# Eurus-Holmes/VAG-NMT

Measured on AMD Instinct MI355X. Metric: training sentence-pairs/sec (Multi30K en->de, B=64), higher is better.
Workload: dtype f32; 1 GPU; configs[1]: multimodal en->de train step, B=64/GPU, Ts=Tt=40, E=256, H=512, S=512, I=2048, Vs=8507, V=9391, dropout 0.3/0.5/0.5, tied emb, teacher_force_ratio=1; global_batch=64, parallelism=dp1, hip_graph=True

## Files before the change

vag-nmt_amd/csrc/api.hip:

```cpp
#include "../../include/vag_nmt.h"
#include "api_shared.h"
#include <cstring>

static thread_local VagCallCtx g_base_ctx;
static thread_local VagCallCtx* g_active_ctx = nullptr;
VagCallCtx& vag_ctx() { return g_active_ctx ? *g_active_ctx : g_base_ctx; }
VagCallScope::VagCallScope(VagCallCtx& c) : ctx(c), prev(g_active_ctx) { g_active_ctx = &c; }
VagCallScope::~VagCallScope() {
    (void)vag_loss_defer_flush();
    if (ctx.leaf_on) vag_leaf_drop();
    g_active_ctx = prev;
}

VagOptions& vag_opt() {
    static VagOptions o;
    return o;
}

int vag_version(void) { return 330; }

int vag_set_option(const char* name, int64_t value) {
    VAG_CHECK_ARG(name != nullptr);
    VagOptions& o = vag_opt();
    const struct { const char* n; int* p; } ints[] = {
// ... 545 lines not shown
    return vag_surface_expand_launch(rows, R, L, off, chars, V, out, C, lens, S_(stream));
}
int vag_chrf_supported(int64_t Nh, int64_t Ch, int64_t Nr, int64_t Cr) { return vag_chrf_supported_host(Nh, Ch, Nr, Cr); }
int vag_chrf_max_chars(void) { return vag_chrf_max_chars_host(); }
int vag_chrf_select(const int32_t* hchars, const int32_t* hlens, const int32_t* rchars, const int32_t* rlens, const float* weights,
                    int64_t B, int64_t Nh, int64_t Ch, int64_t Nr, int64_t Cr, int32_t* matches, float* util, float* expected,
                    int64_t* best, vag_stream_t stream) {
    return vag_chrf_select_launch(hchars, hlens, rchars, rlens, weights, B, Nh, Ch, Nr, Cr, matches, util, expected, best, S_(stream));
}

int vag_mrt_weights(const float* nll, const float* cost, const float* valid, int64_t B, int64_t Tt, int64_t N, float alpha, float scale,
                    float* inv_cnt, float* q, float* risk, vag_stream_t stream) {
    VAG_CHECK_ARG(risk != nullptr);
    return vag_mrt_weights_launch(nll, cost, valid, B, Tt, N, alpha, scale, inv_cnt, q, risk, nullptr, 0.f, 0, S_(stream));
}
int vag_mrt_pack(const int64_t* cand, int64_t G, int64_t Nc, int64_t L, const int64_t* gold, int64_t Tg, int include_gold, int64_t* tgt,
                 int64_t Tt, float* valid, vag_stream_t stream) {
    return vag_mrt_pack_launch(cand, G, Nc, L, gold, Tg, include_gold, tgt, Tt, valid, S_(stream));
}

int vag_clip_adam_flat(float* p, float* g, float* m, float* v, int64_t n, int nseg, const int64_t* seg_off,
                       const float* seg_lr, const float* seg_wd, float clip, float grad_scale, float beta1, float beta2,
                       float eps, int zero_grad, int32_t* step, float* norm_out, void* scratch, const float* lr_dev,
                       vag_stream_t stream) {
    return vag_clip_adam_launch(p, g, m, v, n, nseg, seg_off, seg_lr, seg_wd, clip, grad_scale, beta1, beta2, eps, zero_grad,
                                step, norm_out, scratch, lr_dev, S_(stream));
}

int vag_clip_adam_flat_ema(float* p, float* g, float* m, float* v, int64_t n, int nseg, const int64_t* seg_off,
                           const float* seg_lr, const float* seg_wd, float clip, float grad_scale, float beta1, float beta2,
                           float eps, int zero_grad, int32_t* step, float* norm_out, void* scratch, const float* lr_dev,
                           float* ema, float ema_decay, int ema_warmup, vag_stream_t stream) {
    return vag_clip_adam_ema_launch(p, g, m, v, n, nseg, seg_off, seg_lr, seg_wd, clip, grad_scale, beta1, beta2, eps, zero_grad,
                                    step, norm_out, scratch, lr_dev, ema, ema_decay, ema_warmup, S_(stream));
}

int vag_swap_flat(float* a, float* b, int64_t n, vag_stream_t stream) { return vag_swap_flat_launch(a, b, n, S_(stream)); }

int vag_clip_adam_shard(float* p, float* g, float* m, float* v, int64_t n, int nseg, const int64_t* seg_off, const float* seg_lr,
                        const float* seg_wd, float clip, float grad_scale, float beta1, float beta2, float eps, int zero_grad,
                        int32_t* step, float* norm_out, void* scratch, const float* lr_dev, int64_t lo, int64_t hi, int phase,
                        double* sumsq, vag_stream_t stream) {
    return vag_clip_adam_shard_launch(p, g, m, v, n, nseg, seg_off, seg_lr, seg_wd, clip, grad_scale, beta1, beta2, eps, zero_grad,
                                      step, norm_out, scratch, lr_dev, lo, hi, phase, sumsq, S_(stream));
}

int vag_copy4(const void* const* src, void* const* dst, const int64_t* bytes, int n, vag_stream_t stream) {
    return vag_copy4_launch(src, dst, bytes, n, S_(stream));
}

int vag_recurrence_supported(int kind, int64_t B, int64_t Ts, int64_t Tt, int64_t H) {
    if (kind == 0) return vag_enc_persistent_ok(B, Ts, H) ? 1 : 0;
    if (kind == 1) return vag_dec_persistent_ok(B, Ts, Tt, H) ? 1 : 0;
    return 0;
}
int vag_persistent_timeouts(void) { return vag_persistent_timeouts_read(); }
int vag_attn_energy_probe(const float* a, const float* b, int64_t n, float* out, vag_stream_t stream) {
    return vag_attn_energy_probe_launch(a, b, n, out, S_(stream));
}
int64_t vag_handoff_planes_floats(int64_t B, int64_t Ts, int64_t Tt, int64_t H) {
    const int64_t e = vag_enc_bwd_planes_floats(B, Ts, H), d = vag_dec_bwd_planes_floats(B, Tt, H);
    const int64_t f = vag_enc_fwd_planes_floats(B, Ts, H) + vag_dec_fwd_planes_floats(B, Tt, H);
    return std::max(std::max(e, d), f);
}
int vag_set_handoff_planes(float* buf, int64_t floats) {
    VAG_CHECK_ARG((buf == nullptr || (floats > 0 && aligned16(buf))));
    g_base_ctx.handoff_planes = buf;
    g_base_ctx.handoff_floats = buf ? floats : 0;
    return VAG_OK;
}
int vag_set_operator_guard(void* guard) {
    VAG_CHECK_ARG((reinterpret_cast<uintptr_t>(guard) & 3) == 0);
    g_base_ctx.guard = reinterpret_cast<unsigned*>(guard);
    return VAG_OK;
}
int vag_gemm_group_plan(int n, const int64_t* M, const int64_t* N, const int64_t* K, const int* accumulate, int* split,
                        int* order) {
    return vag_gemm_group_plan_host(n, M, N, K, accumulate, split, order);
}
int vag_gemm_plan(int64_t M, int64_t N, int64_t K, int a_kc, int b_kc, int vec, float beta, int act, int c_half, int a_bf16,
                  int rowsum, int planes, int* plan) {
    return vag_gemm_plan_host(M, N, K, a_kc, b_kc, vec, beta, act, c_half, a_bf16, rowsum, planes, plan);
}
int vag_recurrence_time(int kind, double* ms_total, int* launches) { return vag_persistent_time_read(kind, ms_total, launches); }
int64_t vag_recurrence_sync_words(int kind, int64_t B, int64_t T) {
    return kind == 0 ? vag_enc_persistent_sync_words(B, T) : vag_dec_persistent_sync_words(B, T);
}
int vag_dropout_mask(const uint64_t* rng, int which, int64_t n, float p, float* out, vag_stream_t stream) {
    VAG_CHECK_ARG(which >= 1 && which <= 3);
    return vag_dropout_mask_launch(rng, which, n, p, out, S_(stream));
}
int vag_rng_advance(uint64_t* rng, vag_stream_t stream) { return vag_rng_advance_launch(rng, S_(stream)); }
```

vag-nmt_amd/csrc/persist.hip:

```cpp
#include "kernels.h"
#include "gemm_shared.h"
#include <algorithm>
#include <atomic>
#include <mutex>

namespace {

typedef unsigned __attribute__((address_space(1))) gu32;
#define RLX_AGENT __ATOMIC_RELAXED, __HIP_MEMORY_SCOPE_AGENT

constexpr unsigned SPIN_LIMIT = 1u << 19;
__device__ unsigned g_persist_timeouts;
__device__ unsigned g_persist_guard[2];
__device__ __forceinline__ void note_timeout(unsigned* err, unsigned* guard) {
    __hip_atomic_store((gu32*)err, 1u, RLX_AGENT);
    __hip_atomic_store((gu32*)guard, 1u, RLX_AGENT);
    atomicAdd(guard + 1, 1u);
    atomicAdd(&g_persist_timeouts, 1u);
}

struct EncPArgs {
    const float* xp;
    const float* W[2];
    const float* bias[2];
    const int* lengths;
    float* hst;
    float* gates;
    float* enc;
    unsigned* cnt;
    unsigned* err;
    unsigned* guard;
    unsigned spin;
    const uint64_t* rng;
    float p_ctx;
    int B, Ts, H, RT, CS;
    int rt0, RTP;
    char* pl;
};

template <int N> __device__ __forceinline__ void ld_rows_sc1(const float* p, float4 (&a)[N], float4 (&b)[N]);
template <> __device__ __forceinline__ void ld_rows_sc1<1>(const float* p, float4 (&a)[1], float4 (&b)[1]) {
    asm volatile("global_load_dwordx4 %0, %2, off sc1\n\tglobal_load_dwordx4 %1, %2, off offset:16 sc1\n\ts_waitcnt vmcnt(0)"
                 : "=&v"(a[0]), "=&v"(b[0]) : "v"(p) : "memory");
}
template <> __device__ __forceinline__ void ld_rows_sc1<2>(const float* p, float4 (&a)[2], float4 (&b)[2]) {
    asm volatile("global_load_dwordx4 %0, %4, off sc1\n\tglobal_load_dwordx4 %1, %4, off offset:16 sc1\n\t"
                 "global_load_dwordx4 %2, %4, off offset:128 sc1\n\tglobal_load_dwordx4 %3, %4, off offset:144 sc1\n\t"
                 "s_waitcnt vmcnt(0)"
                 : "=&v"(a[0]), "=&v"(b[0]), "=&v"(a[1]), "=&v"(b[1]) : "v"(p) : "memory");
}
template <> __device__ __forceinline__ void ld_rows_sc1<3>(const float* p, float4 (&a)[3], float4 (&b)[3]) {
    asm volatile("global_load_dwordx4 %0, %6, off sc1\n\tglobal_load_dwordx4 %1, %6, off offset:16 sc1\n\t"
                 "global_load_dwordx4 %2, %6, off offset:128 sc1\n\tglobal_load_dwordx4 %3, %6, off offset:144 sc1\n\t"
                 "global_load_dwordx4 %4, %6, off offset:256 sc1\n\tglobal_load_dwordx4 %5, %6, off offset:272 sc1\n\t"
                 "s_waitcnt vmcnt(0)"
                 : "=&v"(a[0]), "=&v"(b[0]), "=&v"(a[1]), "=&v"(b[1]), "=&v"(a[2]), "=&v"(b[2]) : "v"(p) : "memory");
}
template <> __device__ __forceinline__ void ld_rows_sc1<4>(const float* p, float4 (&a)[4], float4 (&b)[4]) {
    asm volatile("global_load_dwordx4 %0, %8, off sc1\n\tglobal_load_dwordx4 %1, %8, off offset:16 sc1\n\t"
                 "global_load_dwordx4 %2, %8, off offset:128 sc1\n\tglobal_load_dwordx4 %3, %8, off offset:144 sc1\n\t"
                 "global_load_dwordx4 %4, %8, off offset:256 sc1\n\tglobal_load_dwordx4 %5, %8, off offset:272 sc1\n\t"
                 "global_load_dwordx4 %6, %8, off offset:384 sc1\n\tglobal_load_dwordx4 %7, %8, off offset:400 sc1\n\t"
// ... 517 lines not shown
    unsigned* err;
    unsigned* guard;
    unsigned spin;
    int B, Ts, H, RT, CS;
    int rt0, RTP;
    char* pl;
};
template <int KS, bool PL>
__global__ __launch_bounds__(512, 1) void enc_bwd_persistent_kernel(EncBArgs a) {
    __shared__ __attribute__((aligned(16))) float lds[21504];
    const int wg = blockIdx.x;
    const int cs = wg % a.CS, rt = a.rt0 + (wg / a.CS) % a.RTP, d = wg / (a.CS * a.RTP);
    const int lane = threadIdx.x & 63, wave = threadIdx.x >> 6;
    const int H = a.H, B = a.B, Ts = a.Ts, K = 3 * H;
    const int m0 = rt * 16, u0 = cs * 16;
    const int fr = lane & 15, fg = lane >> 4;
    const int kbase = wave * (K >> 3);
    const int64_t BH = (int64_t)B * H;
    bf16x8 wf[KS][3];
    {
        const float* WT = a.WT[d] + (int64_t)(u0 + fr) * K + kbase + 8 * fg;
#pragma unroll
        for (int s = 0; s < KS; ++s) split8(*reinterpret_cast<const float4*>(WT + 32 * s), *reinterpret_cast<const float4*>(WT + 32 * s + 4), wf[s]);
    }
    const int erow = lane >> 2, equad = lane & 3, eslot = erow + 16 * equad;
    const int em = m0 + erow, eu = u0 + 4 * equad;
    const bool eok = wave == 0 && em < B;
    const int len = eok ? a.lengths[em] : 0;
    float4 carry = make_float4(0.f, 0.f, 0.f, 0.f);
    float* dghd = a.dgh + (int64_t)d * Ts * B * K;
    const char* pld = PL ? a.pl + ((int64_t)d * Ts * a.RT + rt) * pl_block_bytes(K) : nullptr;
    const int64_t pl_step = (int64_t)a.RT * pl_block_bytes(K);
    const int pl_ld = __builtin_amdgcn_readfirstlane(wave) * KS * PL_KSTEP_BYTES;
    const int pl_st = (u0 >> 5) * PL_KSTEP_BYTES, pl_gate = (H >> 5) * PL_KSTEP_BYTES;
    const unsigned pl_so = pl_slot_off(lane >> 2, u0 + 4 * (lane & 3));
    gu32* cnt = (gu32*)(a.cnt + ((int64_t)d * a.RT + rt) * Ts);
    const int lrow = min(m0 + ld_row(lane), B - 1);
    const int src4 = ld_src4(lane);
    float4* red = reinterpret_cast<float4*>(lds);
    bool dead = false;
    const int64_t ld_add = (int64_t)Ts * 2 * H;

    for (int k = Ts - 1; k >= 0; --k) {
        const int t = d == 0 ? k : Ts - 1 - k;
        float4 sv[4], hp, e4;
        if (eok) {
            const int64_t o = (int64_t)em * H + eu;
            const float* g = a.gates + ((int64_t)(d * Ts + k) * 4) * BH + o;
#pragma unroll
            for (int q = 0; q < 4; ++q) sv[q] = *reinterpret_cast<const float4*>(g + q * BH);
            hp = *reinterpret_cast<const float4*>(a.hst + ((int64_t)d * (Ts + 1) + k) * BH + o);
            e4 = *reinterpret_cast<const float4*>(a.d_enc + (int64_t)em * ld_add + (int64_t)t * 2 * H + d * H + eu);
        }
        float4 dh = carry;
        if (k < Ts - 1) {
            if (threadIdx.x == 0 && !dead) {
                unsigned spins = 0;
                while (__hip_atomic_load(cnt + (k + 1), RLX_AGENT) < (unsigned)a.CS) {
                    if (++spins > a.spin) { note_timeout(a.err, a.guard); dead = true; break; }
                }
            }
            __syncthreads();
            f32x4 acc = {0.f, 0.f, 0.f, 0.f};
            if (PL) {
                u32x4 gf[3 * KS];
                ld_planes_sc1<KS>(pld + (k + 1) * pl_step + pl_ld, 16u * lane, gf);
                acc = mma6_planes<KS>(wf, gf, acc);
            } else {
                float4 ga[KS], gb[KS];
                ld_rows_sc1<KS>(dghd + ((int64_t)(k + 1) * B + lrow) * K + kbase + 8 * (lane & 3), ga, gb);
#pragma unroll
                for (int s = 0; s < KS; ++s) {
                    bf16x8 hf[3];
                    split8(perm4(ga[s], src4), perm4(gb[s], src4), hf);
                    acc = mma6(wf[s], hf, acc);
                }
            }
            red[wave * 64 + lane] = make_float4(acc[0], acc[1], acc[2], acc[3]);
            __syncthreads();
            if (wave == 0) {
#pragma unroll
                for (int w = 0; w < 8; ++w) {
                    const float4 o = red[w * 64 + eslot];
                    dh.x += o.x; dh.y += o.y; dh.z += o.z; dh.w += o.w;
                }
            }
        }
        if (PL && wave == 0 && !eok) {
#pragma unroll
            for (int g = 0; g < 3; ++g) st_planes4(pld + k * pl_step + pl_st + g * pl_gate, pl_so, make_float4(0.f, 0.f, 0.f, 0.f));
        }
        if (eok) {
            const bool active = t < len;
            float dhv[4] = {dh.x, dh.y, dh.z, dh.w};
            float gi[3][4], gh[3][4], cy[4];
            if (!active) {
#pragma unroll
                for (int q = 0; q < 4; ++q) { gi[0][q] = gi[1][q] = gi[2][q] = gh[0][q] = gh[1][q] = gh[2][q] = 0.f; cy[q] = dhv[q]; }
            } else {
                const float ev[4] = {e4.x, e4.y, e4.z, e4.w};
                const float r_[4] = {sv[0].x, sv[0].y, sv[0].z, sv[0].w}, z_[4] = {sv[1].x, sv[1].y, sv[1].z, sv[1].w};
                const float n_[4] = {sv[2].x, sv[2].y, sv[2].z, sv[2].w}, hn[4] = {sv[3].x, sv[3].y, sv[3].z, sv[3].w};
                const float hpv[4] = {hp.x, hp.y, hp.z, hp.w};
#pragma unroll
                for (int q = 0; q < 4; ++q) {
                    float e = ev[q];
                    if (a.rng && a.p_ctx > 0.f)
                        e *= vag_drop_mul(a.rng, VAG_DROP_ENC_CTX, (uint64_t)em * ld_add + (uint64_t)t * 2 * H + d * H + eu + q, a.p_ctx);
                    const float x = dhv[q] + e;
                    const float dn_pre = x * (1.f - z_[q]) * (1.f - n_[q] * n_[q]);
                    const float dz_pre = x * (hpv[q] - n_[q]) * z_[q] * (1.f - z_[q]);
                    const float dr_pre = dn_pre * hn[q] * r_[q] * (1.f - r_[q]);
                    gi[0][q] = dr_pre; gi[1][q] = dz_pre; gi[2][q] = dn_pre;
                    gh[0][q] = dr_pre; gh[1][q] = dz_pre; gh[2][q] = dn_pre * r_[q];
                    cy[q] = x * z_[q];
                }
            }
            carry = make_float4(cy[0], cy[1], cy[2], cy[3]);
            float* gho = dghd + ((int64_t)k * B + em) * K + eu;
#pragma unroll
            for (int g = 0; g < 3; ++g) {
                const float4 x = make_float4(gh[g][0], gh[g][1], gh[g][2], gh[g][3]);
                if (PL) st_planes4(pld + k * pl_step + pl_st + g * pl_gate, pl_so, x);
                else st_sc1_f4(gho + g * H, x);
            }
            asm volatile("s_waitcnt vmcnt(0)" ::: "memory");
            if (lane == 0) __hip_atomic_fetch_add(cnt + k, 1u, RLX_AGENT);
            if (PL) {
#pragma unroll
                for (int g = 0; g < 3; ++g) *reinterpret_cast<float4*>(gho + g * H) = make_float4(gh[g][0], gh[g][1], gh[g][2], gh[g][3]);
            }
            float* gio = a.d_xp + ((int64_t)t * B + em) * 6 * H + d * 3 * H + eu;
#pragma unroll
            for (int g = 0; g < 3; ++g) *reinterpret_cast<float4*>(gio + g * H) = make_float4(gi[g][0], gi[g][1], gi[g][2], gi[g][3]);
        }
    }
}

struct EncWBArgs {
    const vag_half* WT16[2];
    const float* d_enc;
    const float* gates;
    const float* hst;
    const int* lengths;
    const uint64_t* rng; float p_ctx;
    float* d_xp;
    float* dgh;
    vag_half* gx;
    unsigned* cnt;
    unsigned* err;
    unsigned* guard;
    unsigned spin;
    int B, Ts, H, RG, CS;
};
template <> __device__ __forceinline__ void ld16_sc1<6>(const vag_half* p, u32x4 (&v)[6]) {
    asm volatile("global_load_dwordx4 %0, %6, off sc1\n\tglobal_load_dwordx4 %1, %6, off offset:64 sc1\n\t"
                 "global_load_dwordx4 %2, %6, off offset:128 sc1\n\tglobal_load_dwordx4 %3, %6, off offset:192 sc1\n\t"
                 "global_load_dwordx4 %4, %6, off offset:256 sc1\n\tglobal_load_dwordx4 %5, %6, off offset:320 sc1\n\t"
                 "s_waitcnt vmcnt(0)"
                 : "=&v"(v[0]), "=&v"(v[1]), "=&v"(v[2]), "=&v"(v[3]), "=&v"(v[4]), "=&v"(v[5]) : "v"(p) : "memory");
}
// ... 208 lines not shown
                 "global_load_dwordx4 %10, %28, off offset:128 sc1\n\tglobal_load_dwordx4 %11, %28, off offset:144 sc1\n\t"
                 "global_load_dwordx4 %12, %28, off offset:256 sc1\n\tglobal_load_dwordx4 %13, %28, off offset:272 sc1\n\t"
                 "global_load_dwordx4 %14, %28, off offset:384 sc1\n\tglobal_load_dwordx4 %15, %28, off offset:400 sc1\n\t"
                 "global_load_dwordx4 %16, %28, off offset:512 sc1\n\tglobal_load_dwordx4 %17, %28, off offset:528 sc1\n\t"
                 "global_load_dwordx4 %18, %28, off offset:640 sc1\n\tglobal_load_dwordx4 %19, %28, off offset:656 sc1\n\t"
                 "s_waitcnt vmcnt(0)"
                 : "=&v"(a0), "=&v"(a1), "=&v"(a2), "=&v"(a3), "=&v"(b0), "=&v"(b1), "=&v"(b2), "=&v"(b3),
                   "=&v"(a[0]), "=&v"(b[0]), "=&v"(a[1]), "=&v"(b[1]), "=&v"(a[2]), "=&v"(b[2]), "=&v"(a[3]), "=&v"(b[3]),
                   "=&v"(a[4]), "=&v"(b[4]), "=&v"(a[5]), "=&v"(b[5])
                 : "v"(p0), "v"(p01), "v"(p02), "v"(p03), "v"(p1), "v"(p11), "v"(p12), "v"(p13), "v"(rows) : "memory");
    v0 = (a0 + a1) + (a2 + a3);
    v1 = (b0 + b1) + (b2 + b3);
}

__device__ __forceinline__ void ld_acc_shards_and_rows3(const float* p0, const float* p1, int64_t stride, float& v0, float& v1,
                                                        const float* rows, float4 (&a)[3], float4 (&b)[3]) {
    float a0, a1, a2, a3, b0, b1, b2, b3;
    const float *p02 = p0 + 2 * stride, *p12 = p1 + 2 * stride;
    const float *p01 = p0 + stride, *p03 = p02 + stride, *p11 = p1 + stride, *p13 = p12 + stride;
    asm volatile("global_load_dword %0, %14, off sc1\n\tglobal_load_dword %1, %15, off sc1\n\t"
                 "global_load_dword %2, %16, off sc1\n\tglobal_load_dword %3, %17, off sc1\n\t"
                 "global_load_dword %4, %18, off sc1\n\tglobal_load_dword %5, %19, off sc1\n\t"
                 "global_load_dword %6, %20, off sc1\n\tglobal_load_dword %7, %21, off sc1\n\t"
                 "global_load_dwordx4 %8, %22, off sc1\n\tglobal_load_dwordx4 %9, %22, off offset:16 sc1\n\t"
                 "global_load_dwordx4 %10, %22, off offset:128 sc1\n\tglobal_load_dwordx4 %11, %22, off offset:144 sc1\n\t"
                 "global_load_dwordx4 %12, %22, off offset:256 sc1\n\tglobal_load_dwordx4 %13, %22, off offset:272 sc1\n\t"
                 "s_waitcnt vmcnt(0)"
                 : "=&v"(a0), "=&v"(a1), "=&v"(a2), "=&v"(a3), "=&v"(b0), "=&v"(b1), "=&v"(b2), "=&v"(b3),
                   "=&v"(a[0]), "=&v"(b[0]), "=&v"(a[1]), "=&v"(b[1]), "=&v"(a[2]), "=&v"(b[2])
                 : "v"(p0), "v"(p01), "v"(p02), "v"(p03), "v"(p1), "v"(p11), "v"(p12), "v"(p13), "v"(rows) : "memory");
    v0 = (a0 + a1) + (a2 + a3);
    v1 = (b0 + b1) + (b2 + b3);
}
__device__ __forceinline__ void ld_acc_shards_and_rows(const float* p0, const float* p1, int64_t stride, float& v0, float& v1,
                                                       const float* rows, float4 (&a)[6], float4 (&b)[6]) {
    ld_acc_shards_and_rows6(p0, p1, stride, v0, v1, rows, a, b);
}
__device__ __forceinline__ void ld_acc_shards_and_rows(const float* p0, const float* p1, int64_t stride, float& v0, float& v1,
                                                       const float* rows, float4 (&a)[3], float4 (&b)[3]) {
    ld_acc_shards_and_rows3(p0, p1, stride, v0, v1, rows, a, b);
}

constexpr int DEC_WGS = 64;
template <int WGS>
__device__ __forceinline__ void dec_slice_map(int mode, int rt0, int& i, int& rt) {
    const int bx = blockIdx.x % WGS;
    rt = rt0 + blockIdx.x / WGS;
    int g = mode == 1 ? 8 : (mode == 2 ? 2 : (mode == 3 ? 4 : 1));
    if (g > WGS / 8) g = WGS / 8;
    i = (bx & 7) * g + ((bx >> 3) % g) + 8 * g * (bx / (8 * g));
}
constexpr int ACC_SHARDS = 4;
constexpr int DEC_U = 8;

constexpr int DEC_E = 4 * DEC_WGS;
__device__ __forceinline__ unsigned long long cand_key(float v, int idx) {
    const unsigned u = __builtin_bit_cast(unsigned, v);
    return ((unsigned long long)(u ^ ((u >> 31) ? 0xffffffffu : 0x80000000u)) << 32) | (unsigned long long)(0xffffffffu - (unsigned)idx);
}

template <bool FREE, int WGS = DEC_WGS, bool PL = false>
__global__ __launch_bounds__(512, 1) void dec_fwd_persistent_kernel(DecPArgs a) {
    extern __shared__ __attribute__((aligned(16))) float dlds[];
    static_assert(WGS == 64 || (WGS == 32 && !FREE), "H = 512 (both forms) or H = 256 (teacher-forced form)");
    static_assert(!(PL && FREE), "the free-running form keeps the fp32 hand-off");
    constexpr int H = WGS * DEC_U, C = 2 * H, Q = C + 3 * H, KS = H / 256;
    constexpr int E = DEC_E;
    int i, rt;
    dec_slice_map<WGS>(a.xcd_map, a.rt0, i, rt);
    const int lane = threadIdx.x & 63, wave = threadIdx.x >> 6;
    const int B = a.B, Ts = a.Ts, Tt = a.Tt;
    const int m0 = rt * 16, u0 = i * DEC_U;
    const int fr = lane & 15, fg = lane >> 4;
    const int kbase = wave * (H >> 3);
    const int64_t BH = (int64_t)B * H;
    float4* red = reinterpret_cast<float4*>(dlds);
    float* pe_s = dlds + 6144;
    float* ew_s = pe_s + 16 * Ts * 16;
    float* sc_s = ew_s + 16 * Ts * 24;
    float* gi_s = sc_s + 16 * Ts;
    float* hp_s = gi_s + 16 * 24;
    float* bs_s = hp_s + 16 * 24;
    float* hs_s = bs_s + 80;
    float* v_s = hs_s + 256;
    float* mk_s = v_s + C;
    float* q_s = mk_s + 16 * Ts;
    float* cw_s = q_s + 256;
    float* hb_s = cw_s + 64;
    int* tok_s = reinterpret_cast<int*>(hb_s + 16);
    float* ew2_s = reinterpret_cast<float*>(tok_s + 16);
    unsigned long long* cb_s = reinterpret_cast<unsigned long long*>(q_s);
    bf16x8* tm_s = reinterpret_cast<bf16x8*>(red);

#ifdef VAG_LAB
#define VAG_PSTAMP(k) do { if (!FREE && a.dbg && blockIdx.x == 0 && threadIdx.x == 0) a.dbg[Tt * 8 + (k)] = __builtin_amdgcn_s_memrealtime(); } while (0)
#else
#define VAG_PSTAMP(k) do { } while (0)
#endif
    VAG_PSTAMP(0);
#ifdef VAG_LAB
    if (!FREE && a.dbg && threadIdx.x == 0 && rt < 8) {
        if (i == 0) a.dbg[(Tt + 1) * 8 + rt] = __builtin_amdgcn_s_memrealtime();
        if (i == WGS - 1) a.dbg[(Tt + 3) * 8 + rt] = __builtin_amdgcn_s_memrealtime();
    }
#endif
    bf16x8 w1[KS][2][3], w2[KS][3][3];
// ... 373 lines not shown
                    ho[q] = (1.f - zz[q]) * nn[q] + zz[q] * hpv[q];
                }
                const float4 h1v = tag4(make_float4(ho[0], ho[1], ho[2], ho[3]));
                *reinterpret_cast<float4*>(hs_s + fr * 8 + 4 * hq) = h1v;
                const int64_t o = (int64_t)em * H + eu;
                st_sc1_f4(a.h1 + (int64_t)t * BH + o, h1v);
                if (!VAG_TAGGED) asm volatile("s_waitcnt vmcnt(0)" ::: "memory");
                if (VAG_TAGGED && tx == 0) arrive(c2 + t * CNT_WORDS, i);
                float* sv = a.g1 + (int64_t)t * 4 * BH + o;
                *reinterpret_cast<float4*>(sv) = make_float4(rr[0], rr[1], rr[2], rr[3]);
                *reinterpret_cast<float4*>(sv + BH) = make_float4(zz[0], zz[1], zz[2], zz[3]);
                *reinterpret_cast<float4*>(sv + 2 * BH) = make_float4(nn[0], nn[1], nn[2], nn[3]);
                *reinterpret_cast<float4*>(sv + 3 * BH) = make_float4(gh[0], gh[1], gh[2], gh[3]);
            }
            if (tx == 0 && (!VAG_TAGGED || !eok)) arrive(c2 + t * CNT_WORDS, i);
        }
        VAG_STAMP(2);
        wait_count(c2 + t * CNT_WORDS, PER_SHARD, a.err, a.guard, a.spin, dead);
        VAG_STAMP(3);
        bf16x8 hf2[KS][3];
        if constexpr (PL) {
            u32x4 gf[3 * KS];
            ld_planes_marked<KS>(plb + t * pl_step + pl_ld, 16u * lane, gf, a.spin, dead, a.err, a.guard);
#pragma unroll
            for (int s = 0; s < 3 * KS; ++s) hf2[s / 3][s % 3] = __builtin_bit_cast(bf16x8, gf[s]);
        } else {
            ld_rows_tagged<KS>(a.h1 + ((int64_t)t * B + lrow) * H + kbase + 8 * (lane & 3), ha, hb, a.spin, dead, a.err, a.guard);
#pragma unroll
            for (int s = 0; s < KS; ++s) { ha[s] = perm4(ha[s], src4); hb[s] = perm4(hb[s], src4); }
        }
        {
            f32x4 acc = {0.f, 0.f, 0.f, 0.f};
#pragma unroll
            for (int s = 0; s < KS; ++s) {
                if constexpr (!PL) split8(ha[s], hb[s], hf2[s]);
                acc = mma6(w2[s][0], hf2[s], acc);
            }
            red[(wave * 3 + 0) * 64 + lane] = make_float4(acc[0], acc[1], acc[2], acc[3]);
        }
        __syncthreads();
        if (wave == 0) {
            float4 qv = make_float4(0, 0, 0, 0);
#pragma unroll
            for (int w = 0; w < 8; ++w) {
                const float4 x0 = red[(w * 3 + 0) * 64 + lane];
                qv.x += x0.x; qv.y += x0.y; qv.z += x0.z; qv.w += x0.w;
            }
            if (m0 + fr < B) *reinterpret_cast<float4*>(a.qhp + ((int64_t)t * B + m0 + fr) * Q + 16 * i + 4 * fg) = qv;
            *reinterpret_cast<float4*>(q_s + fr * 16 + 4 * fg) =
                make_float4(vag_energy_exp(qv.x), vag_energy_exp(qv.y), vag_energy_exp(qv.z), vag_energy_exp(qv.w));
        }
        __syncthreads();
        {
            const int cq = tx & 3;
            const float4 vq = *reinterpret_cast<const float4*>(v_s + 16 * i + 4 * cq);
            for (int P = tx >> 2; P < 16 * Ts; P += 128) {
                const int r = P / Ts;
                const float4 pv = reinterpret_cast<const float4*>(pe_s)[P * 4 + cq];
                const float4 qq = *reinterpret_cast<const float4*>(q_s + r * 16 + 4 * cq);
                float acc = vq.x * vag_energy_tanh(pv.x, qq.x) + vq.y * vag_energy_tanh(pv.y, qq.y) + vq.z * vag_energy_tanh(pv.z, qq.z) +
                            vq.w * vag_energy_tanh(pv.w, qq.w);
                acc = quad_sum(acc);
                if (cq == 0 && m0 + r < B)
                    atomicAdd(a.psc + (((int64_t)t * ACC_SHARDS + (i & (ACC_SHARDS - 1))) * B + m0 + r) * Ts + (P - r * Ts), acc);
            }
        }
        {
            f32x4 acc[2] = {{0.f, 0.f, 0.f, 0.f}, {0.f, 0.f, 0.f, 0.f}};
#pragma unroll
            for (int s = 0; s < KS; ++s) {
                acc[0] = mma6(w2[s][1], hf2[s], acc[0]);
                acc[1] = mma6(w2[s][2], hf2[s], acc[1]);
            }
            red[(wave * 3 + 1) * 64 + lane] = make_float4(acc[0][0], acc[0][1], acc[0][2], acc[0][3]);
            red[(wave * 3 + 2) * 64 + lane] = make_float4(acc[1][0], acc[1][1], acc[1][2], acc[1][3]);
        }
        VAG_STAMP(4);
        asm volatile("s_waitcnt vmcnt(0)" ::: "memory");
        __syncthreads();
        if (tx == 0) arrive(c4 + t * CNT_WORDS, i);
        VAG_STAMP(5);
        if (ep) {
            float4 hp2[3] = {make_float4(0, 0, 0, 0), make_float4(0, 0, 0, 0), make_float4(0, 0, 0, 0)};
#pragma unroll
            for (int w = 0; w < 8; ++w) {
                const float4 x0 = red[(w * 3 + 1) * 64 + hq * 16 + fr], x1 = red[(w * 3 + 1) * 64 + (2 + hq) * 16 + fr];
                const float4 x2 = red[(w * 3 + 2) * 64 + hq * 16 + fr];
                hp2[0].x += x0.x; hp2[0].y += x0.y; hp2[0].z += x0.z; hp2[0].w += x0.w;
                hp2[1].x += x1.x; hp2[1].y += x1.y; hp2[1].z += x1.z; hp2[1].w += x1.w;
                hp2[2].x += x2.x; hp2[2].y += x2.y; hp2[2].z += x2.z; hp2[2].w += x2.w;
            }
#pragma unroll
            for (int g = 0; g < 3; ++g) {
                const float4 bb = *reinterpret_cast<const float4*>(bs_s + 24 + g * 8 + 4 * hq);
                hp2[g].x += bb.x; hp2[g].y += bb.y; hp2[g].z += bb.z; hp2[g].w += bb.w;
                *reinterpret_cast<float4*>(hp_s + fr * 24 + g * 8 + 4 * hq) = hp2[g];
                if (eok) *reinterpret_cast<float4*>(a.qhp + ((int64_t)t * B + em) * Q + C + g * H + eu) = hp2[g];
            }
        }
        VAG_STAMP(6);
        wait_count(c4 + t * CNT_WORDS, PER_SHARD, a.err, a.guard, a.spin, dead);
        VAG_STAMP(7);
        for (int x0 = tx; x0 < 16 * Ts; x0 += 1024) {
            const int x1 = x0 + 512;
            const int r0 = x0 / Ts, r1 = min(x1, 16 * Ts - 1) / Ts;
            const float* p0 = a.psc + ((int64_t)t * ACC_SHARDS * B + min(m0 + r0, B - 1)) * Ts + (x0 - r0 * Ts);
            const float* p1 = a.psc + ((int64_t)t * ACC_SHARDS * B + min(m0 + r1, B - 1)) * Ts + (min(x1, 16 * Ts - 1) - r1 * Ts);
            float v0, v1;
            ld_acc_shards(p0, p1, (int64_t)B * Ts, v0, v1);
            sc_s[x0] = mk_s[x0] == 0.f ? -INFINITY : v0;
            if (x1 < 16 * Ts) sc_s[x1] = mk_s[x1] == 0.f ? -INFINITY : v1;
        }
        __syncthreads();
        for (int r = wave; r < 16; r += 8) {
            float mx = -INFINITY;
            for (int sp = lane; sp < Ts; sp += 64) mx = fmaxf(mx, sc_s[r * Ts + sp]);
            mx = wave_max(mx);
            float sum = 0.f;
            for (int sp = lane; sp < Ts; sp += 64) sum += __expf(sc_s[r * Ts + sp] - mx);
            sum = wave_sum(sum);
            const float inv = 1.f / sum;
            for (int sp = lane; sp < Ts; sp += 64) {
                const float al = __expf(sc_s[r * Ts + sp] - mx) * inv;
                sc_s[r * Ts + sp] = al;
                if (((r * Ts + sp) & (WGS - 1)) == i && m0 + r < B) a.alpha[((int64_t)t * B + m0 + r) * Ts + sp] = al;
            }
        }
        __syncthreads();
        if (tx < 16 * 24) {
            const int r = tx / 24, col = tx - r * 24;
            const float* al = sc_s + r * Ts;
            const float* ew = ew_s + (int64_t)r * Ts * 24 + col;
            float s0 = 0.f, s1 = 0.f;
            int sp = 0;
            for (; sp + 1 < Ts; sp += 2) { s0 += al[sp] * ew[sp * 24]; s1 += al[sp + 1] * ew[(sp + 1) * 24]; }
            if (sp < Ts) s0 += al[sp] * ew[sp * 24];
            gi_s[tx] = s0 + s1;
        } else if (FREE && tx < 16 * 24 + 64) {
            const int x = tx - 16 * 24, r = x >> 2, col = x & 3;
            const float* al = sc_s + r * Ts;
            const float* ew = ew2_s + (int64_t)r * Ts * 4 + col;
            float s0 = 0.f, s1 = 0.f;
            int sp = 0;
            for (; sp + 1 < Ts; sp += 2) { s0 += al[sp] * ew[sp * 4]; s1 += al[sp + 1] * ew[(sp + 1) * 4]; }
            if (sp < Ts) s0 += al[sp] * ew[sp * 4];
            cw_s[x] = s0 + s1;
        }
        __syncthreads();
        if constexpr (PL) {
            if (ep2 && !eok2) st_planes2_marked(plb + (Tt + t) * pl_step + pl_st, pl_so + 4 * eh, 0.f, 0.f);
            if (eok2) {
                const int e8 = 4 * hq + 2 * eh;
                float gi[3][2], bi[3][2], hh[3][2];
#pragma unroll
                for (int g = 0; g < 3; ++g) {
                    const float2 x = *reinterpret_cast<const float2*>(gi_s + fr * 24 + g * 8 + e8);
                    const float2 y = *reinterpret_cast<const float2*>(bs_s + 48 + g * 8 + e8);
                    const float2 z = *reinterpret_cast<const float2*>(hp_s + fr * 24 + g * 8 + e8);
                    gi[g][0] = x.x; gi[g][1] = x.y;
                    bi[g][0] = y.x; bi[g][1] = y.y;
                    hh[g][0] = z.x; hh[g][1] = z.y;
                }
                const float2 h1v = *reinterpret_cast<const float2*>(hs_s + fr * 8 + e8);
                const float h1a[2] = {h1v.x, h1v.y};
                float rr[2], zz[2], nn[2], ho[2];
#pragma unroll
                for (int q = 0; q < 2; ++q) {
                    rr[q] = vag_sigmoid(gi[0][q] + bi[0][q] + hh[0][q]);
                    zz[q] = vag_sigmoid(gi[1][q] + bi[1][q] + hh[1][q]);
                    nn[q] = vag_tanh(gi[2][q] + bi[2][q] + rr[q] * hh[2][q]);
                    ho[q] = (1.f - zz[q]) * nn[q] + zz[q] * h1a[q];
                }
                const float2 h2v = make_float2(tag1(ho[0]), tag1(ho[1]));
                *reinterpret_cast<float2*>(hs_s + 128 + fr * 8 + e8) = h2v;
                st_planes2_marked(plb + (Tt + t) * pl_step + pl_st, pl_so + 4 * eh, h2v.x, h2v.y);
                if (tx == 0) arrive(c1 + t * CNT_WORDS, i);
                const int64_t o = (int64_t)em * H + eu2;
                *reinterpret_cast<float2*>(a.h2_all + (int64_t)t * BH + o) = h2v;
                float* sv = a.g2 + (int64_t)t * 4 * BH + o;
                *reinterpret_cast<float2*>(sv) = make_float2(rr[0], rr[1]);
                *reinterpret_cast<float2*>(sv + BH) = make_float2(zz[0], zz[1]);
                *reinterpret_cast<float2*>(sv + 2 * BH) = make_float2(nn[0], nn[1]);
                *reinterpret_cast<float2*>(sv + 3 * BH) = make_float2(hh[2][0], hh[2][1]);
            }
            if (tx == 0 && !eok2) arrive(c1 + t * CNT_WORDS, i);
        }
        if (!PL && eok) {
            float gi[3][4];
#pragma unroll
            for (int g = 0; g < 3; ++g) {
                const float4 x = *reinterpret_cast<const float4*>(gi_s + fr * 24 + g * 8 + 4 * hq);
                gi[g][0] = x.x; gi[g][1] = x.y; gi[g][2] = x.z; gi[g][3] = x.w;
            }
            float bi[3][4], hh[3][4];
#pragma unroll
            for (int g = 0; g < 3; ++g) {
                const float4 x = *reinterpret_cast<const float4*>(bs_s + 48 + g * 8 + 4 * hq);
                const float4 y = *reinterpret_cast<const float4*>(hp_s + fr * 24 + g * 8 + 4 * hq);
                bi[g][0] = x.x; bi[g][1] = x.y; bi[g][2] = x.z; bi[g][3] = x.w;
// ... 180 lines not shown
    auto red4 = [&](float (&x)[4]) {
        float4 sum = red[hq * 16 + fr];
#pragma unroll
        for (int w = 1; w < 8; ++w) {
            const float4 o = red[w * 64 + hq * 16 + fr];
            sum.x += o.x; sum.y += o.y; sum.z += o.z; sum.w += o.w;
        }
        x[0] = sum.x; x[1] = sum.y; x[2] = sum.z; x[3] = sum.w;
    };
    auto hid_load = [&](int t, int c, bf16x8 (&wf)[3][3], u32x4 (&gf)[9]) {
        unsigned w2o = pl_w2_off;
        asm volatile("" : "+v"(w2o));
        const char* pw = pl_w2 + w2o;
#pragma unroll
        for (int s = 0; s < 3; ++s)
#pragma unroll
            for (int p = 0; p < 3; ++p)
                wf[s][p] = *reinterpret_cast<const bf16x8*>(pw + (3 * c + s) * PL_W2_KSTEP_BYTES + p * PL_W2_PLANE_BYTES);
        ld_planes_sc1<3>(pl_g2 + t * pl_g1_step + KC * pl_wave + c * (3 * PL_KSTEP_BYTES), 16u * lane, gf);
    };

    VAG_BPSTAMP(1);
    if (ep) {
        if (eok) {
            const float4 d = *reinterpret_cast<const float4*>(a.d_h2_all + (int64_t)(Tt - 1) * BH + (int64_t)em * H + eu);
            const float dh2[4] = {d.x, d.y, d.z, d.w};
            const int64_t o = (int64_t)em * H + eu;
            float4 sv[4];
#pragma unroll
            for (int q = 0; q < 4; ++q) sv[q] = *reinterpret_cast<const float4*>(a.g2 + ((int64_t)(Tt - 1) * 4 + q) * BH + o);
            cell2_bwd(Tt - 1, dh2, sv, *reinterpret_cast<const float4*>(a.h1 + (int64_t)(Tt - 1) * BH + o));
        } else {
#pragma unroll
            for (int g = 0; g < 3; ++g) *reinterpret_cast<float4*>(gi_s + fr * 24 + g * 8 + 4 * hq) = make_float4(0.f, 0.f, 0.f, 0.f);
            *reinterpret_cast<float4*>(d1_s + fr * 8 + 4 * hq) = make_float4(0.f, 0.f, 0.f, 0.f);
            if (PL2) {
#pragma unroll
                for (int g = 0; g < 3; ++g) st_planes4(pl_g2 + (Tt - 1) * pl_g1_step + pl_st_g1 + g * pl_gate, pl_so_g1, make_float4(0.f, 0.f, 0.f, 0.f));
            }
        }
    }
    __syncthreads();

#ifdef VAG_LAB
    const bool stamp = a.dbg != nullptr && blockIdx.x == 0 && threadIdx.x == 0;
#define VAG_STAMP(k) do { if (stamp) a.dbg[t * 8 + (k)] = __builtin_amdgcn_s_memrealtime(); } while (0)
#else
#define VAG_STAMP(k) do { } while (0)
#endif
    for (int t = Tt - 1; t >= 0; --t) {
        int emL = em;
        if (PL) asm volatile("" : "+v"(emL));
        VAG_STAMP(0);
        for (int P = threadIdx.x; P < NP; P += 512) {
            const int r = P / Ts;
            const float* g = gi_s + r * 24;
            float acc = 0.f;
#pragma unroll
            for (int k = 0; k < 24; ++k) acc += ew_t[k * NP + P] * g[k];
            if (m0 + r < B)
                atomicAdd(a.dal + (((int64_t)t * ACC_SHARDS + (i & (ACC_SHARDS - 1))) * B + m0 + r) * Ts + (P - r * Ts), acc);
        }
        asm volatile("s_waitcnt vmcnt(0)" ::: "memory");
        __syncthreads();
        if (threadIdx.x == 0) arrive(cA + t * CNT_WORDS, i);
        if (PL2 && eok) {
#pragma unroll
            for (int g = 0; g < 3; ++g) *reinterpret_cast<float4*>(a.dqgh + ((int64_t)t * B + emL) * Q + C + g * H + eu) = gh2k[g];
        }
        VAG_STAMP(1);
        float4 hga[PL2 ? 1 : KC], hgb[PL2 ? 1 : KC];
        bf16x8 wf0[3][3];
        u32x4 gf0[9];
        static_assert(KC == 6 || KC == 3, "ld_acc_shards_and_rows<KC>, chunks of three k-steps");
        float al0 = 0.f, al1 = 0.f, dh0 = 0.f, dh1_ = 0.f;
        const int x0 = threadIdx.x, x1 = threadIdx.x + 512;
        {
            const int r0 = min(x0, NP - 1) / Ts, r1 = min(x1, NP - 1) / Ts;
            const int64_t o0 = ((int64_t)t * B + min(m0 + r0, B - 1)) * Ts + (min(x0, NP - 1) - r0 * Ts);
            const int64_t o1 = ((int64_t)t * B + min(m0 + r1, B - 1)) * Ts + (min(x1, NP - 1) - r1 * Ts);
            al0 = a.alpha[o0]; dh0 = a.dah[o0];
            if (x1 < NP) { al1 = a.alpha[o1]; dh1_ = a.dah[o1]; }
            const float qv = a.qhp[((int64_t)t * B + min(m0 + (int)((threadIdx.x & 255) >> 4), B - 1)) * Q + 16 * i + (threadIdx.x & 15)];
            wait_count(cA + t * CNT_WORDS, PER_SHARD, a.err, a.guard, a.spin, dead);
            VAG_STAMP(2);
            float v0, v1;
            const float* p0 = a.dal + o0 + (int64_t)t * (ACC_SHARDS - 1) * B * Ts;
            const float* p1 = a.dal + o1 + (int64_t)t * (ACC_SHARDS - 1) * B * Ts;
            if constexpr (PL2) ld_acc_shards(p0, p1, (int64_t)B * Ts, v0, v1);
            else ld_acc_shards_and_rows(p0, p1, (int64_t)B * Ts, v0, v1,
                                        a.dqgh + ((int64_t)t * B + lrow) * Q + C + wave * (3 * H >> 3) + 8 * (lane & 3), hga, hgb);
            if (x0 < NP) { da_s[x0] = v0 + dh0; al_s[x0] = al0; }
            if (x1 < NP) { da_s[x1] = v1 + dh1_; al_s[x1] = al1; }
            __syncthreads();
            for (int r = wave; r < 16; r += 8) {
                float dot = 0.f;
                for (int sp = lane; sp < Ts; sp += 64) dot += al_s[r * Ts + sp] * da_s[r * Ts + sp];
                dot = wave_sum(dot);
                for (int sp = lane; sp < Ts; sp += 64) {
                    const float d = al_s[r * Ts + sp] * (da_s[r * Ts + sp] - dot);
                    da_s[r * Ts + sp] = d;
                    if (((r * Ts + sp) & (WGS - 1)) == i && m0 + r < B) a.ds[((int64_t)t * B + m0 + r) * Ts + sp] = d;
                }
            }
            __syncthreads();
            {
                const int tt = threadIdx.x & 255, half = threadIdx.x >> 8;
                const int r = tt >> 4, c = tt & 15;
                const float* pr = pe_s + (int64_t)r * Ts * 16 + c;
                const float* dsr = da_s + r * Ts;
                float acc0 = 0.f, acc1 = 0.f;
                int sp = half;
                const float eq = vag_energy_exp(qv);
                for (; sp + 2 < Ts; sp += 4) {
                    const float r0 = vag_energy_rcp(pr[sp * 16], eq), r1 = vag_energy_rcp(pr[(sp + 2) * 16], eq);
                    acc0 = __builtin_fmaf(dsr[sp], __builtin_fmaf(-r0, r0, r0), acc0);
                    acc1 = __builtin_fmaf(dsr[sp + 2], __builtin_fmaf(-r1, r1, r1), acc1);
                }
                if (sp < Ts) { const float r0 = vag_energy_rcp(pr[sp * 16], eq); acc0 = __builtin_fmaf(dsr[sp], __builtin_fmaf(-r0, r0, r0), acc0); }
                float* half_s = reinterpret_cast<float*>(red);
                if (half) half_s[tt] = acc0 + acc1;
                __syncthreads();
                if (!half) dq_s[tt] = ((acc0 + acc1) + half_s[tt]) * vq4;
            }
            __syncthreads();
            if constexpr (PL2) {
                const int r = (threadIdx.x >> 2) & 15, c4 = threadIdx.x & 3;
                const bool w0 = threadIdx.x < 64;
                float4 dqv = make_float4(0.f, 0.f, 0.f, 0.f);
                if (w0) {
                    dqv = *reinterpret_cast<const float4*>(dq_s + r * 16 + 4 * c4);
                    st_planes4(pl_dq + t * pl_dq_step + pl_st_dq, pl_so_dq, m0 + r < B ? dqv : make_float4(0.f, 0.f, 0.f, 0.f));
                }
                hid_load(t, 0, wf0, gf0);
                if (threadIdx.x == 0) arrive(cB + t * CNT_WORDS, i);
                if (w0 && m0 + r < B) *reinterpret_cast<float4*>(a.dqgh + ((int64_t)t * B + m0 + r) * Q + 16 * i + 4 * c4) = dqv;
            } else if (threadIdx.x < 64) {
                const int r = threadIdx.x >> 2, c4 = threadIdx.x & 3;
                const float4 dqv = *reinterpret_cast<const float4*>(dq_s + r * 16 + 4 * c4);
                float* dqo = a.dqgh + ((int64_t)t * B + m0 + r) * Q + 16 * i + 4 * c4;
                if (PL) st_planes4(pl_dq + t * pl_dq_step + pl_st_dq, pl_so_dq, m0 + r < B ? dqv : make_float4(0.f, 0.f, 0.f, 0.f));
                else if (m0 + r < B) st_sc1_f4(dqo, dqv);
                asm volatile("s_waitcnt vmcnt(0)" ::: "memory");
                if (threadIdx.x == 0) arrive(cB + t * CNT_WORDS, i);
                if (PL && m0 + r < B) *reinterpret_cast<float4*>(dqo) = dqv;
            }
        }
        VAG_STAMP(3);
        {
            f32x4 acc = {0.f, 0.f, 0.f, 0.f};
            if constexpr (PL2) {
                acc = mma6_planes<3>(wf0, gf0, acc);
#pragma unroll
                for (int c = 1; c < KC / 3; ++c) {
                    hid_load(t, c, wf0, gf0);
                    acc = mma6_planes<3>(wf0, gf0, acc);
                }
            } else {
#pragma unroll
                for (int s = 0; s < KC; ++s) {
                    bf16x8 wf[3], hf[3];
                    split8(perm4(*reinterpret_cast<const float4*>(wa_row + 32 * s), src4),
                           perm4(*reinterpret_cast<const float4*>(wa_row + 32 * s + 4), src4), wf);
                    split8(perm4(hga[s], src4), perm4(hgb[s], src4), hf);
                    acc = mma6(wf, hf, acc);
                }
// ... 614 lines not shown
```

Baseline: 23340 sentence-pairs/s.

## Batch LDS loads and software-pipeline attention loops in persistent decoder kernels

Measured after the change: 23970 sentence-pairs/s, median of 6. +2.7%, better.

```diff
diff --git a/vag-nmt_amd/csrc/api.hip b/vag-nmt_amd/csrc/api.hip
--- a/vag-nmt_amd/csrc/api.hip
+++ b/vag-nmt_amd/csrc/api.hip
@@ -621,6 +621,7 @@
 int vag_recurrence_supported(int kind, int64_t B, int64_t Ts, int64_t Tt, int64_t H) {
     if (kind == 0) return vag_enc_persistent_ok(B, Ts, H) ? 1 : 0;
     if (kind == 1) return vag_dec_persistent_ok(B, Ts, Tt, H) ? 1 : 0;
+    if (kind == 2) return vag_dec_bwd_persistent_ok(B, Ts, Tt, H) ? 1 : 0;
     return 0;
 }
 int vag_persistent_timeouts(void) { return vag_persistent_timeouts_read(); }
diff --git a/vag-nmt_amd/csrc/persist.hip b/vag-nmt_amd/csrc/persist.hip
--- a/vag-nmt_amd/csrc/persist.hip
+++ b/vag-nmt_amd/csrc/persist.hip
@@ -8,6 +8,18 @@
 
 typedef unsigned __attribute__((address_space(1))) gu32;
 #define RLX_AGENT __ATOMIC_RELAXED, __HIP_MEMORY_SCOPE_AGENT
+
+__device__ __forceinline__ void pin4(float (&x)[4]) { asm volatile("" : "+v"(x[0]), "+v"(x[1]), "+v"(x[2]), "+v"(x[3])); }
+__device__ __forceinline__ void pin6(float (&x)[6]) {
+    asm volatile("" : "+v"(x[0]), "+v"(x[1]), "+v"(x[2]), "+v"(x[3]), "+v"(x[4]), "+v"(x[5]));
+}
+__device__ __forceinline__ void pin8(float (&x)[8]) {
+    asm volatile("" : "+v"(x[0]), "+v"(x[1]), "+v"(x[2]), "+v"(x[3]), "+v"(x[4]), "+v"(x[5]), "+v"(x[6]), "+v"(x[7]));
+}
+__device__ __forceinline__ void pin12(float (&x)[12]) {
+    asm volatile("" : "+v"(x[0]), "+v"(x[1]), "+v"(x[2]), "+v"(x[3]), "+v"(x[4]), "+v"(x[5]), "+v"(x[6]), "+v"(x[7]), "+v"(x[8]),
+                      "+v"(x[9]), "+v"(x[10]), "+v"(x[11]));
+}
 
 constexpr unsigned SPIN_LIMIT = 1u << 19;
 __device__ unsigned g_persist_timeouts;
@@ -631,6 +643,13 @@
             hp = *reinterpret_cast<const float4*>(a.hst + ((int64_t)d * (Ts + 1) + k) * BH + o);
             e4 = *reinterpret_cast<const float4*>(a.d_enc + (int64_t)em * ld_add + (int64_t)t * 2 * H + d * H + eu);
         }
+        float dm[4] = {1.f, 1.f, 1.f, 1.f};
+        if (eok && a.rng && a.p_ctx > 0.f) {
+#pragma unroll
+            for (int q = 0; q < 4; ++q)
+                dm[q] = vag_drop_mul(a.rng, VAG_DROP_ENC_CTX, (uint64_t)em * ld_add + (uint64_t)t * 2 * H + d * H + eu + q, a.p_ctx);
+            pin4(dm);
+        }
         float4 dh = carry;
         if (k < Ts - 1) {
             if (threadIdx.x == 0 && !dead) {
@@ -683,9 +702,9 @@
                 const float hpv[4] = {hp.x, hp.y, hp.z, hp.w};
 #pragma unroll
                 for (int q = 0; q < 4; ++q) {
+#pragma clang fp contract(off)
                     float e = ev[q];
-                    if (a.rng && a.p_ctx > 0.f)
-                        e *= vag_drop_mul(a.rng, VAG_DROP_ENC_CTX, (uint64_t)em * ld_add + (uint64_t)t * 2 * H + d * H + eu + q, a.p_ctx);
+                    if (a.rng && a.p_ctx > 0.f) e = e * dm[q];
                     const float x = dhv[q] + e;
                     const float dn_pre = x * (1.f - z_[q]) * (1.f - n_[q] * n_[q]);
                     const float dz_pre = x * (hpv[q] - n_[q]) * z_[q] * (1.f - z_[q]);
@@ -1000,6 +1019,31 @@
 }
 constexpr int ACC_SHARDS = 4;
 constexpr int DEC_U = 8;
+
+template <int STRIDE> __device__ __forceinline__ float ctx_dot(const float* al, const float* ew, int Ts) {
+    float s0 = 0.f, s1 = 0.f;
+    int sp = 0;
+    for (; sp + 8 <= Ts; sp += 8) {
+        float x[8], y[8];
+#pragma unroll
+        for (int k = 0; k < 8; ++k) { x[k] = al[sp + k]; y[k] = ew[(sp + k) * STRIDE]; }
+        pin8(x); pin8(y);
+#pragma unroll
+        for (int k = 0; k < 8; k += 2) { s0 = __builtin_fmaf(x[k], y[k], s0); s1 = __builtin_fmaf(x[k + 1], y[k + 1], s1); }
+    }
+    if (sp + 4 <= Ts) {
+        float x[4], y[4];
+#pragma unroll
+        for (int k = 0; k < 4; ++k) { x[k] = al[sp + k]; y[k] = ew[(sp + k) * STRIDE]; }
+        pin4(x); pin4(y);
+        s0 = __builtin_fmaf(x[0], y[0], s0); s1 = __builtin_fmaf(x[1], y[1], s1);
+        s0 = __builtin_fmaf(x[2], y[2], s0); s1 = __builtin_fmaf(x[3], y[3], s1);
+        sp += 4;
+    }
+    for (; sp + 1 < Ts; sp += 2) { s0 = __builtin_fmaf(al[sp], ew[sp * STRIDE], s0); s1 = __builtin_fmaf(al[sp + 1], ew[(sp + 1) * STRIDE], s1); }
+    if (sp < Ts) s0 = __builtin_fmaf(al[sp], ew[sp * STRIDE], s0);
+    return s0 + s1;
+}
 
 constexpr int DEC_E = 4 * DEC_WGS;
 __device__ __forceinline__ unsigned long long cand_key(float v, int idx) {
@@ -1479,17 +1523,34 @@
         }
         __syncthreads();
         {
-            const int cq = tx & 3;
+            int txs = tx;
+            asm volatile("" : "+v"(txs));
+            const int cq = txs & 3;
             const float4 vq = *reinterpret_cast<const float4*>(v_s + 16 * i + 4 * cq);
-            for (int P = tx >> 2; P < 16 * Ts; P += 128) {
-                const int r = P / Ts;
+            float* psc_t = a.psc + (((int64_t)t * ACC_SHARDS + (i & (ACC_SHARDS - 1))) * B + m0) * Ts;
+            const int NPf = 16 * Ts, PV = (B - m0) * Ts;
+            const int dq_ = 128 / Ts, dr_ = 128 - dq_ * Ts;
+            int P = txs >> 2, r = P / Ts, s = P - r * Ts;
+            float pq[8] = {0.f, 0.f, 0.f, 0.f, 0.f, 0.f, 0.f, 0.f};
+            auto request = [&]() {
                 const float4 pv = reinterpret_cast<const float4*>(pe_s)[P * 4 + cq];
                 const float4 qq = *reinterpret_cast<const float4*>(q_s + r * 16 + 4 * cq);
-                float acc = vq.x * vag_energy_tanh(pv.x, qq.x) + vq.y * vag_energy_tanh(pv.y, qq.y) + vq.z * vag_energy_tanh(pv.z, qq.z) +
-                            vq.w * vag_energy_tanh(pv.w, qq.w);
+                pq[0] = pv.x; pq[1] = pv.y; pq[2] = pv.z; pq[3] = pv.w; pq[4] = qq.x; pq[5] = qq.y; pq[6] = qq.z; pq[7] = qq.w;
+            };
+            if (P < NPf) request();
+            while (P < NPf) {
+                float c[8];
+#pragma unroll
+                for (int k = 0; k < 8; ++k) c[k] = pq[k];
+                const int Pc = P;
+                P += 128; r += dq_; s += dr_;
+                if (s >= Ts) { s -= Ts; ++r; }
+                if (P < NPf) request();
+                __builtin_amdgcn_sched_barrier(0);
+                float acc = vq.x * vag_energy_tanh(c[0], c[4]) + vq.y * vag_energy_tanh(c[1], c[5]) + vq.z * vag_energy_tanh(c[2], c[6]) +
+                            vq.w * vag_energy_tanh(c[3], c[7]);
                 acc = quad_sum(acc);
-                if (cq == 0 && m0 + r < B)
-                    atomicAdd(a.psc + (((int64_t)t * ACC_SHARDS + (i & (ACC_SHARDS - 1))) * B + m0 + r) * Ts + (P - r * Ts), acc);
+                if (cq == 0 && Pc < PV) atomicAdd(psc_t + Pc, acc);
             }
         }
         {
@@ -1539,7 +1600,23 @@
             if (x1 < 16 * Ts) sc_s[x1] = mk_s[x1] == 0.f ? -INFINITY : v1;
         }
         __syncthreads();
-        for (int r = wave; r < 16; r += 8) {
+        if (Ts <= 64) {
+            int txm = tx;
+            asm volatile("" : "+v"(txm));
+            const int ln = txm & 63, wv = txm >> 6;
+            const bool on = ln < Ts;
+            const int x0 = wv * Ts + ln, x1 = x0 + 8 * Ts;
+            const float a0 = on ? sc_s[x0] : -INFINITY, a1 = on ? sc_s[x1] : -INFINITY;
+            const float mx0 = wave_max(a0), mx1 = wave_max(a1);
+            const float e0 = on ? __expf(a0 - mx0) : 0.f, e1 = on ? __expf(a1 - mx1) : 0.f;
+            const float sum0 = wave_sum(e0), sum1 = wave_sum(e1);
+            const float al0 = e0 * (1.f / sum0), al1 = e1 * (1.f / sum1);
+            if (on) {
+                sc_s[x0] = al0; sc_s[x1] = al1;
+                if ((x0 & (WGS - 1)) == i && m0 + wv < B) a.alpha[((int64_t)t * B + m0 + wv) * Ts + ln] = al0;
+                if ((x1 & (WGS - 1)) == i && m0 + wv + 8 < B) a.alpha[((int64_t)t * B + m0 + wv + 8) * Ts + ln] = al1;
+            }
+        } else for (int r = wave; r < 16; r += 8) {
             float mx = -INFINITY;
             for (int sp = lane; sp < Ts; sp += 64) mx = fmaxf(mx, sc_s[r * Ts + sp]);
             mx = wave_max(mx);
@@ -1556,22 +1633,10 @@
         __syncthreads();
         if (tx < 16 * 24) {
             const int r = tx / 24, col = tx - r * 24;
-            const float* al = sc_s + r * Ts;
-            const float* ew = ew_s + (int64_t)r * Ts * 24 + col;
-            float s0 = 0.f, s1 = 0.f;
-            int sp = 0;
-            for (; sp + 1 < Ts; sp += 2) { s0 += al[sp] * ew[sp * 24]; s1 += al[sp + 1] * ew[(sp + 1) * 24]; }
-            if (sp < Ts) s0 += al[sp] * ew[sp * 24];
-            gi_s[tx] = s0 + s1;
+            gi_s[tx] = ctx_dot<24>(sc_s + r * Ts, ew_s + r * Ts * 24 + col, Ts);
         } else if (FREE && tx < 16 * 24 + 64) {
             const int x = tx - 16 * 24, r = x >> 2, col = x & 3;
-            const float* al = sc_s + r * Ts;
-            const float* ew = ew2_s + (int64_t)r * Ts * 4 + col;
-            float s0 = 0.f, s1 = 0.f;
-            int sp = 0;
-            for (; sp + 1 < Ts; sp += 2) { s0 += al[sp] * ew[sp * 4]; s1 += al[sp + 1] * ew[(sp + 1) * 4]; }
-            if (sp < Ts) s0 += al[sp] * ew[sp * 4];
-            cw_s[x] = s0 + s1;
+            cw_s[x] = ctx_dot<4>(sc_s + r * Ts, ew2_s + r * Ts * 4 + col, Ts);
         }
         __syncthreads();
         if constexpr (PL) {
@@ -1858,14 +1923,49 @@
         int emL = em;
         if (PL) asm volatile("" : "+v"(emL));
         VAG_STAMP(0);
-        for (int P = threadIdx.x; P < NP; P += 512) {
-            const int r = P / Ts;
-            const float* g = gi_s + r * 24;
-            float acc = 0.f;
-#pragma unroll
-            for (int k = 0; k < 24; ++k) acc += ew_t[k * NP + P] * g[k];
-            if (m0 + r < B)
-                atomicAdd(a.dal + (((int64_t)t * ACC_SHARDS + (i & (ACC_SHARDS - 1))) * B + m0 + r) * Ts + (P - r * Ts), acc);
+        {
+            float* dal_t = a.dal + (((int64_t)t * ACC_SHARDS + (i & (ACC_SHARDS - 1))) * B + m0) * Ts;
+            const int PV = (B - m0) * Ts;
+            int txA = threadIdx.x;
+            asm volatile("" : "+v"(txA));
+            const int rest = NP & 511, nwhole = rest > 384 ? NP : NP - rest;
+            for (int P = txA; P < nwhole; P += 512) {
+                float s0 = 0.f, s1 = 0.f;
+                const int r = P / Ts;
+#pragma unroll
+                for (int hb = 0; hb < 2; ++hb) {
+                    float e[12], g[12];
+#pragma unroll
+                    for (int k = 0; k < 12; ++k) e[k] = ew_t[(12 * hb + k) * NP + P];
+#pragma unroll
+                    for (int k = 0; k < 12; k += 4) {
+                        const float4 g4 = *reinterpret_cast<const float4*>(gi_s + r * 24 + 12 * hb + k);
+                        g[k] = g4.x; g[k + 1] = g4.y; g[k + 2] = g4.z; g[k + 3] = g4.w;
+                    }
+                    pin12(e); pin12(g);
+#pragma unroll
+                    for (int k = 0; k < 12; k += 2) { s0 = __builtin_fmaf(e[k], g[k], s0); s1 = __builtin_fmaf(e[k + 1], g[k + 1], s1); }
+                }
+                if (P < PV) atomicAdd(dal_t + P, s0 + s1);
+            }
+            const int qd = txA & 3;
+            for (int P = nwhole + (txA >> 2); P < NP; P += 128) {
+                const int r = P / Ts;
+                float e[6], g[6];
+#pragma unroll
+                for (int k = 0; k < 6; ++k) e[k] = ew_t[(6 * qd + k) * NP + P];
+#pragma unroll
+                for (int k = 0; k < 6; k += 2) {
+                    const float2 g2 = *reinterpret_cast<const float2*>(gi_s + r * 24 + 6 * qd + k);
+                    g[k] = g2.x; g[k + 1] = g2.y;
+                }
+                pin6(e); pin6(g);
+                float s0 = e[0] * g[0], s1 = e[1] * g[1];
+#pragma unroll
+                for (int k = 2; k < 6; k += 2) { s0 = __builtin_fmaf(e[k], g[k], s0); s1 = __builtin_fmaf(e[k + 1], g[k + 1], s1); }
+                const float acc = quad_sum(s0 + s1);
+                if (qd == 0 && P < PV) atomicAdd(dal_t + P, acc);
+            }
         }
         asm volatile("s_waitcnt vmcnt(0)" ::: "memory");
         __syncthreads();
@@ -1899,7 +1999,21 @@
             if (x0 < NP) { da_s[x0] = v0 + dh0; al_s[x0] = al0; }
             if (x1 < NP) { da_s[x1] = v1 + dh1_; al_s[x1] = al1; }
             __syncthreads();
-            for (int r = wave; r < 16; r += 8) {
+            if (Ts <= 64) {
+                int txm = threadIdx.x;
+                asm volatile("" : "+v"(txm));
+                const int ln = txm & 63, wv = txm >> 6;
+                const bool on = ln < Ts;
+                const int y0 = wv * Ts + ln, y1 = y0 + 8 * Ts;
+                const float a0 = on ? al_s[y0] : 0.f, a1 = on ? al_s[y1] : 0.f, g0 = on ? da_s[y0] : 0.f, g1 = on ? da_s[y1] : 0.f;
+                const float dot0 = wave_sum(on ? __builtin_fmaf(a0, g0, 0.f) : 0.f), dot1 = wave_sum(on ? __builtin_fmaf(a1, g1, 0.f) : 0.f);
+                if (on) {
+                    const float d0 = a0 * (g0 - dot0), d1 = a1 * (g1 - dot1);
+                    da_s[y0] = d0; da_s[y1] = d1;
+                    if ((y0 & (WGS - 1)) == i && m0 + wv < B) a.ds[((int64_t)t * B + m0 + wv) * Ts + ln] = d0;
+                    if ((y1 & (WGS - 1)) == i && m0 + wv + 8 < B) a.ds[((int64_t)t * B + m0 + wv + 8) * Ts + ln] = d1;
+                }
+            } else for (int r = wave; r < 16; r += 8) {
                 float dot = 0.f;
                 for (int sp = lane; sp < Ts; sp += 64) dot += al_s[r * Ts + sp] * da_s[r * Ts + sp];
                 dot = wave_sum(dot);
@@ -1918,6 +2032,31 @@
                 float acc0 = 0.f, acc1 = 0.f;
                 int sp = half;
                 const float eq = vag_energy_exp(qv);
+                for (; sp + 14 < Ts; sp += 16) {
+                    float x[8], y[8];
+#pragma unroll
+                    for (int k = 0; k < 8; ++k) { x[k] = pr[(sp + 2 * k) * 16]; y[k] = dsr[sp + 2 * k]; }
+                    pin8(x); pin8(y);
+#pragma unroll
+                    for (int k = 0; k < 8; k += 2) {
+                        const float r0 = vag_energy_rcp(x[k], eq), r1 = vag_energy_rcp(x[k + 1], eq);
+                        acc0 = __builtin_fmaf(y[k], __builtin_fmaf(-r0, r0, r0), acc0);
+                        acc1 = __builtin_fmaf(y[k + 1], __builtin_fmaf(-r1, r1, r1), acc1);
+                    }
+                }
+                if (sp + 6 < Ts) {
+                    float x[4], y[4];
+#pragma unroll
+                    for (int k = 0; k < 4; ++k) { x[k] = pr[(sp + 2 * k) * 16]; y[k] = dsr[sp + 2 * k]; }
+                    pin4(x); pin4(y);
+#pragma unroll
+                    for (int k = 0; k < 4; k += 2) {
+                        const float r0 = vag_energy_rcp(x[k], eq), r1 = vag_energy_rcp(x[k + 1], eq);
+                        acc0 = __builtin_fmaf(y[k], __builtin_fmaf(-r0, r0, r0), acc0);
+                        acc1 = __builtin_fmaf(y[k + 1], __builtin_fmaf(-r1, r1, r1), acc1);
+                    }
+                    sp += 8;
+                }
                 for (; sp + 2 < Ts; sp += 4) {
                     const float r0 = vag_energy_rcp(pr[sp * 16], eq), r1 = vag_energy_rcp(pr[(sp + 2) * 16], eq);
                     acc0 = __builtin_fmaf(dsr[sp], __builtin_fmaf(-r0, r0, r0), acc0);
```
